# mrinmoy-iitg/SM_HPSS_MTL

Hardware: AMD Instinct MI355X
Metric: clips/sec HPSS+MTL-CNN fwd (1s@16kHz) (higher is better)
Workload: dtype f32

## Files before the change

sm_hpss_mtl_amd/csrc/smh_median.hip:

```cpp
#include <cstdlib>

#include "smh_median_kernel.h"
#include "smh_median_split.h"

namespace smh_median {

const Entry kPairs[] = {
    SMH_MEDIAN_E2(21, 11) SMH_MEDIAN_E2(17, 17)
    SMH_MEDIAN_E2(11, 11) SMH_MEDIAN_E2(11, 21) SMH_MEDIAN_E2(11, 31) SMH_MEDIAN_E2(11, 41) SMH_MEDIAN_E2(11, 51)
    SMH_MEDIAN_E2(21, 21) SMH_MEDIAN_E2(21, 31) SMH_MEDIAN_E2(21, 41) SMH_MEDIAN_E2(21, 51)
    SMH_MEDIAN_E2(31, 11) SMH_MEDIAN_E2(31, 21) SMH_MEDIAN_E2(31, 31) SMH_MEDIAN_E2(31, 41) SMH_MEDIAN_E2(31, 51)
    SMH_MEDIAN_E2(41, 11) SMH_MEDIAN_E2(41, 21) SMH_MEDIAN_E2(41, 31) SMH_MEDIAN_E2(41, 41) SMH_MEDIAN_E2(41, 51)
    SMH_MEDIAN_E2(51, 11) SMH_MEDIAN_E2(51, 21) SMH_MEDIAN_E2(51, 31) SMH_MEDIAN_E2(51, 41) SMH_MEDIAN_E2(51, 51)};

KernelFn find_pair_kernel(int lh, int lp) {
    for (const Entry &e : kPairs)
        if (e.lh == lh && e.lp == lp) return e.fn;
    return nullptr;
}

}

namespace {

// ... 105 lines not shown
    if (best < 0) return false;
    if (const char *ev = getenv("SMH_MEDIAN_SEG")) {
        int a = 0, b = 0;
        if (sscanf(ev, "%d,%d", &a, &b) == 2 && (!lh || a >= 1) && (!lp || b >= 1) &&
            waves(K, lh ? a : 0) + waves(nt, lp ? b : 0) <= maxwaves)
            bh = lh ? a : 0, bp = lp ? b : 0;
    }
    p->nsh = bh, p->nsp = bp, p->nwh = waves(K, bh), p->nwp = waves(nt, bp);
    return true;
}

int launch_small(const float *S, int B, int K, int T, int w, int along_t, float *out, hipStream_t st) {
    const size_t total = (size_t)B * K * T;
    const int bs = 256;
    hipLaunchKernelGGL(median_small_kernel, dim3((unsigned)((total + bs - 1) / bs)), dim3(bs), 0, st, S, out, K, T, w,
                       along_t, total);
    return smh::launch_status("median_small_kernel");
}

enum Family { kFamCopy = 0, kFamSmall = 1, kFamSplit = 2, kFamPersist = 3, kFamDeleteInsert = 4, kFamTwoSingles = 5 };
struct Route {
    int family, layout;
    Plan plan;
    KernelFn fn;
    const SplitEntry *se;
    const PersistEntry *pe;
    int n_cu;
};

int launch_route(int B, int K, int T, int lh, int lp, int harm_tmajor, Route *r) {
    *r = Route{};
    r->layout = harm_tmajor;
    r->fn = (lh && lp) ? find_pair_kernel(lh, lp) : find_single_kernel(lh, lp);
    if (!r->fn) return smh::set_error(SMH_E_INVALID, "no median kernel for (l_harm,l_perc)=(%d,%d)", lh, lp);
    Plan p;
    int rc = make_plan(K, T, lh, lp, &p);
    if (rc) return rc;
    static const bool no_split = getenv("SMH_MEDIAN_NOSPLIT") != nullptr;
    bool want_persist = (lh > 17 || lp > 17);
    if (const char *ev = getenv("SMH_MEDIAN_PERSIST")) want_persist = atoi(ev) != 0;
    int pthreads = 512;
    if (const char *ev = getenv("SMH_MEDIAN_PTHREADS")) pthreads = atoi(ev);
    if (const PersistEntry *pe = (no_split || !want_persist || !(lh && lp)) ? nullptr : find_persist_kernel(lh, lp, pthreads)) {
        static int n_cu = 0;
        if (n_cu == 0) {
            int dev = 0;
            SMH_CHECK_HIP(hipGetDevice(&dev));
            SMH_CHECK_HIP(hipDeviceGetAttribute(&n_cu, hipDeviceAttributeMultiprocessorCount, dev));
        }
        const int tile_bytes = persist_tile_bytes(K, T);
        const int g = T & 63;
        const bool conflict_free = (T & 1) || (g % 4 == 2);
        Plan q = p;
        if (p.ntiles == 1 && conflict_free && 2 * tile_bytes <= smh::kLdsBytesPerCU && B >= 2 * n_cu &&
            make_split_roles(K, T, lh, lp, pe->threads / 64, &q)) {
            r->family = kFamPersist, r->plan = q, r->pe = pe, r->n_cu = n_cu;
            return SMH_OK;
        }
    }
    if (const SplitEntry *se = no_split ? nullptr : find_split_kernel(lh, lp)) {
        Plan q = p;
        if (make_split_roles(K, p.TT, lh, lp, se->threads / 64, &q)) {
            r->family = kFamSplit, r->plan = q, r->se = se;
            return SMH_OK;
        }
    }
    if (harm_tmajor == 2) r->layout = 1;
    r->family = kFamDeleteInsert, r->plan = p;
    return SMH_OK;
}

int launch_routed(const Route &r, const float *S, int B, int K, int T, float *harm, float *perc, hipStream_t st) {
    if (r.family == kFamPersist) {
        const Plan &q = r.plan;
        const int lds = 2 * persist_tile_bytes(K, T);
        SMH_CHECK_HIP(hipFuncSetAttribute((const void *)r.pe->fn, hipFuncAttributeMaxDynamicSharedMemorySize, lds));
        hipLaunchKernelGGL(r.pe->fn, dim3(r.n_cu), dim3((q.nwh + q.nwp) * 64), lds, st, S, harm, perc, B, K, T, q.nsh,
                           q.nsp, q.nwh, r.layout);
        return smh::launch_status("hpss_median_persist_kernel");
    }
    if (r.family == kFamSplit) {
        const Plan &q = r.plan;
        SMH_CHECK_HIP(hipFuncSetAttribute((const void *)r.se->fn, hipFuncAttributeMaxDynamicSharedMemorySize, (int)q.lds));
        dim3 grid(q.ntiles, B), block((q.nwh + q.nwp) * 64);
        const bool probe_noload = smh::probe_env("SMH_MEDIAN_PROBE_NOLOAD") != nullptr;
        hipLaunchKernelGGL(r.se->fn, grid, block, q.lds, st, S, harm, perc, K, T, q.TT, q.stride, q.nsh, q.nsp, q.nwh,
                           r.layout, probe_noload ? 1.f : -__builtin_inff(), __builtin_inff(), nullptr, nullptr, 0);
        return smh::launch_status("hpss_median_split_kernel");
    }
    const Plan &p = r.plan;
    SMH_CHECK_HIP(hipFuncSetAttribute((const void *)r.fn, hipFuncAttributeMaxDynamicSharedMemorySize, (int)p.lds));
    dim3 grid(p.ntiles, B), block((p.nwh + p.nwp) * 64);
    hipLaunchKernelGGL(r.fn, grid, block, p.lds, st, S, harm, perc, K, T, p.TT, p.stride, p.nsh, p.nsp, p.nwh,
                       r.layout, -__builtin_inff(), __builtin_inff());
    return smh::launch_status("hpss_median_kernel");
}

int launch(const float *S, int B, int K, int T, int lh, int lp, float *harm, float *perc, hipStream_t st,
           int harm_tmajor = 0, int *written = nullptr) {
    if (written) *written = harm_tmajor;
    Route r;
    int rc = launch_route(B, K, T, lh, lp, harm_tmajor, &r);
    if (rc) return rc;
    if (written) *written = r.layout;
    return launch_routed(r, S, B, K, T, harm, perc, st);
}

int check_args(const void *S, int B, int K, int T, int w, const char *name) {
    SMH_REQUIRE(S != nullptr || B == 0, "%s: null input", name);
    SMH_REQUIRE(B >= 0 && K >= 1 && T >= 1, "%s: bad shape B=%d K=%d T=%d", name, B, K, T);
    SMH_REQUIRE(w >= 1 && w <= SMH_MAX_MEDIAN && (w & 1), "%s: window must be odd in [1,%d], got %d", name,
                SMH_MAX_MEDIAN, w);
    SMH_REQUIRE(B <= 65535, "%s: B=%d exceeds the grid limit; split the batch", name, B);
    return SMH_OK;
}

bool fast_ok(int n, int w) { return w >= 3 && w / 2 + 4 < n; }

bool pair_fused(int K, int T, int lh, int lp) { return fast_ok(T, lh) && fast_ok(K, lp) && find_pair_kernel(lh, lp); }

int hpss_route(int B, int K, int T, int lh, int lp, int want_tmajor, Route *r) {
    if (pair_fused(K, T, lh, lp)) return launch_route(B, K, T, lh, lp, want_tmajor, r);
    *r = Route{};
    r->family = kFamTwoSingles;
    return SMH_OK;
}

int time_route(int B, int K, int T, int lh, Route *r) {
    if (lh == 1 || !fast_ok(T, lh)) {
        *r = Route{};
        r->family = lh == 1 ? kFamCopy : kFamSmall;
        return SMH_OK;
    }
    return launch_route(B, K, T, lh, 0, 0, r);
}

int time_ex_route(int B, int K, int T, int lh, int harm_layout, Route *r) {
    if (lh == 1 || !fast_ok(T, lh) || harm_layout == 0) return time_route(B, K, T, lh, r);
    return launch_route(B, K, T, lh, 0, harm_layout, r);
}

}

namespace smh_median {
int rag_tile_frames(int K, int lh, int lp, int *stride) {
    static const bool no_split = getenv("SMH_MEDIAN_NOSPLIT") != nullptr;
    if (no_split || !(lh && lp) || !find_split_kernel(lh, lp)) return 0;
    const int hh = lh / 2;
    const int budget_words = (smh::kLdsBytesPerCU / 2 - 1024) / 4;
    int maxcols = budget_words / K;
    if ((maxcols & 1) == 0) maxcols -= 1;
    int TT = (maxcols - 2 * hh) & ~3;
    if (TT < 2 * hh + 8) return 0;
    if (stride) *stride = (TT + 2 * hh) | 1;
    return TT;
}

int launch_rag(const float *d_S, float *d_harm, float *d_perc, int K, int lh, int lp, const smh_rag::Clip *d_clips,
               const smh_rag::Item *d_items, int n_items, hipStream_t st) {
    if (n_items <= 0) return SMH_OK;
    int stride = 0;
    const int TT = rag_tile_frames(K, lh, lp, &stride);
    const SplitEntry *se = TT ? find_split_kernel(lh, lp) : nullptr;
    Plan q;
    if (!se || !make_split_roles(K, TT, lh, lp, se->threads / 64, &q))
        return smh::set_error(SMH_E_INVALID, "ragged medians: no block-split kernel for (l_harm,l_perc)=(%d,%d), K=%d", lh, lp, K);
    const size_t lds = (size_t)K * stride * sizeof(float);
    SMH_CHECK_HIP(hipFuncSetAttribute((const void *)se->fn, hipFuncAttributeMaxDynamicSharedMemorySize, (int)lds));
    const unsigned grid = (unsigned)(8 * (((long long)n_items + 7) / 8));
    hipLaunchKernelGGL(se->fn, dim3(grid), dim3((q.nwh + q.nwp) * 64), lds, st, d_S, d_harm, d_perc, K, 0, TT, stride, q.nsh, q.nsp,
// ... 128 lines not shown
```

sm_hpss_mtl_amd/csrc/smh_median_split.h:

```cpp
#pragma once
#include <cstdint>
#include <type_traits>
#include <utility>

#include "smh_median_kernel.h"
#include "smh_rag.h"

namespace smh_median {

template <int W>
struct SplitTraits {
    static constexpr int H = W / 2;
    static constexpr int lo(int s) { return s - H - 1 > 0 ? s - H - 1 : 0; }
    static constexpr int hi(int s) { return s - 1 < H ? s - 1 : H; }
    static constexpr int off(int s) {
        int o = 0;
        for (int r = 1; r < s; ++r) o += hi(r) - lo(r) + 1;
        return o;
    }
    static constexpr int HIST = off(W);
};

template <int B, int E, typename F>
__device__ __forceinline__ void static_for(F &&f) {
// ... 132 lines not shown
            constexpr int i = decltype(ic)::value;
            constexpr bool has_below = i - 1 >= 0;
            constexpr bool has_above = i <= s - 2;
            constexpr int po = Tr::off(s > 1 ? s - 1 : 1), pl = Tr::lo(s > 1 ? s - 1 : 1);
            const float below = has_below ? h[has_below ? po + (i - 1) - pl : 0] : 0.f;
            const float above = has_above ? h[has_above ? po + i - pl : 0] : 0.f;
            h[Tr::off(s) + i - Tr::lo(s)] = insert_slot<has_below, has_above>(below, x, above);
        });
    });
}

template <int W, int ES>
__device__ __forceinline__ void split_median_walk_blocked(const float *line, int p0, int n_out, int n_steps, int n,
                                                          char *obase, unsigned gk16, unsigned kofs) {
    using Tr = SplitTraits<W>;
    constexpr int H = W / 2, BK = W - 1;
    float e[BK];
    float h[Tr::HIST];
    float pre[H + 1];
    const int plast = p0 + n_out - 1 + H;
    auto load_block = [&](int q0) {
        const int lo = p0 - H + q0;
        const bool interior = (lo >= 0) & (lo + BK <= n) & (lo + BK - 1 <= plast);
        if (__all(interior)) {
            const float *src = line + lo * ES;
            static_for<0, BK>([&](auto uc) { e[decltype(uc)::value] = src[decltype(uc)::value * ES]; });
        } else {
            static_for<0, BK>([&](auto uc) {
                const int pos = min(lo + decltype(uc)::value, plast);
                e[decltype(uc)::value] = line[reflect_hi(reflect_lo(pos), n) * ES];
            });
        }
    };
    load_block(0);
    build_history_b<W>(e, h);
    for (int j0 = 0; j0 < n_steps; j0 += BK) {
        load_block(j0 + BK);
        float o4[4];
        static_for<0, BK>([&](auto pc) {
            constexpr int p = decltype(pc)::value;
            constexpr int b = p + 1, a = BK - p;
            static_for_down<Tr::lo(b), Tr::hi(b) + 1>([&](auto ic) {
                constexpr int i = decltype(ic)::value;
                constexpr bool has_below = i - 1 >= 0;
                constexpr bool has_above = i <= b - 2;
                const float below = has_below ? pre[has_below ? i - 1 : 0] : 0.f;
                const float above = has_above ? pre[i] : 0.f;
                pre[i] = insert_slot<has_below, has_above>(below, e[p], above);
            });
            constexpr int i_lo = (H + 1 - b) > 0 ? (H + 1 - b) : 0;
            constexpr int i_hi = a < H + 1 ? a : H + 1;
            constexpr int ao = Tr::off(a), al = Tr::lo(a);
            float r = 0.f;
            static_for<i_lo, i_hi + 1>([&](auto ic) {
                constexpr int i = decltype(ic)::value;
                float t;
                if constexpr (i == 0) t = pre[H];
                else if constexpr (H - i < 0) t = h[ao + (i - 1) - al];
                else t = fmaxf(h[ao + (i - 1) - al], pre[H - i]);
                r = (i == i_lo) ? t : fminf(r, t);
            });
            o4[p & 3] = r;
            if constexpr ((p & 3) == 3 || p == BK - 1) {
                constexpr int cnt = (p & 3) + 1, pf = p - (p & 3);
                const int j = j0 + pf, t = p0 + j;
                char *dst = obase + (unsigned)(t >> 4) * gk16 + kofs + (unsigned)(t & 15) * 4u;
                if (cnt == 4 && (t & 3) == 0 && j + 3 < n_out) {
                    float4u v = {o4[0], o4[1], o4[2], o4[3]};
                    *reinterpret_cast<float4u *>(dst) = v;
                } else {
#pragma unroll
                    for (int c = 0; c < cnt; ++c) {
                        const int tc = t + c;
                        if (j + c < n_out)
                            *reinterpret_cast<float *>(obase + (unsigned)(tc >> 4) * gk16 + kofs + (unsigned)(tc & 15) * 4u) = o4[c];
                    }
                }
            }
        });
        if (j0 + BK < n_steps) build_history_b<W>(e, h);
    }
}

template <int LH, int LP>
struct SplitCfg {
    static constexpr int kMaxW = LH > LP ? LH : LP;
    static constexpr int kThreads = kMaxW <= 17 ? 512 : 384;
    static constexpr int kWavesPerSimd = kMaxW <= 17 ? 4 : 3;
    static constexpr int kFlatBatch = kMaxW <= 17 ? 20 : 27;
};

template <int LH, int LP>
__global__ void __launch_bounds__((SplitCfg<LH, LP>::kThreads), (SplitCfg<LH, LP>::kWavesPerSimd))
hpss_median_split_kernel(const float *__restrict__ S, float *__restrict__ harm, float *__restrict__ perc, int K, int T,
                         int TT, int stride, int nsh, int nsp, int nwh, int harm_tmajor, float probe, float,
                         const smh_rag::Clip *__restrict__ rag, const smh_rag::Item *__restrict__ items, int n_items) {
    extern __shared__ __attribute__((aligned(16))) float tile[];
    constexpr int HH = LH / 2;
    int b = blockIdx.y, tile_i = blockIdx.x;
    size_t spec_off, harm_off;
    if (rag) {
        const unsigned total = (unsigned)n_items, per_xcd = (total + 7u) >> 3;
        const unsigned j = blockIdx.x >> 3, n = (blockIdx.x & 7u) * per_xcd + j;
        if (j >= per_xcd || n >= total) return;
        const smh_rag::Item item = items[n];
        b = item.clip, tile_i = item.tile;
        T = rag[b].T;
        spec_off = (size_t)rag[b].spec_off, harm_off = (size_t)rag[b].harm_off;
    } else {
        spec_off = (size_t)b * K * T;
        harm_off = harm_tmajor == 2 ? (size_t)b * ((T + 15) >> 4) * K * 16 : spec_off;
    }
    const int t0 = tile_i * TT;
    const int t1 = min(T, t0 + TT);
    const int c0 = max(0, t0 - HH), c1 = min(T, t1 + HH);
    const int ncols = c1 - c0;
    const float *Sb = S + spec_off;
    const int wave = threadIdx.x >> 6, lane = threadIdx.x & 63;
    const int nwaves = blockDim.x >> 6;

    constexpr int kFlatBatch = SplitCfg<LH, LP>::kFlatBatch;
    if (probe > 0.f) {
        for (int i = threadIdx.x; i < K * stride; i += blockDim.x) tile[i] = (float)((i * 2654435761u) >> 8) * (1.0f / 16777216.f);
    } else if (TT >= T && ((K * T) & 1) == 0 && K * T <= kFlatBatch * 2 * (int)blockDim.x) {
        const int n2 = (K * T) >> 1;
        const float2v *src = reinterpret_cast<const float2v *>(Sb);
        const unsigned magic = 0xFFFFFFFFu / (unsigned)T + 1u;
        const int extra = stride - T;
        float2v v[kFlatBatch];
#pragma unroll
        for (int r = 0; r < kFlatBatch; ++r) {
            const int idx = r * (int)blockDim.x + (int)threadIdx.x;
            v[r] = __builtin_nontemporal_load(src + min(idx, n2 - 1));
        }
#pragma unroll
        for (int r = 0; r < kFlatBatch; ++r) {
            const int idx = r * (int)blockDim.x + (int)threadIdx.x;
            if (idx < n2) {
                const unsigned g = 2u * (unsigned)idx;
                const unsigned k0 = __umulhi(g, magic), k1 = __umulhi(g + 1u, magic);
                tile[g + k0 * extra] = v[r].x;
                tile[g + 1u + k1 * extra] = v[r].y;
            }
        }
    } else if (((T | c0 | ncols) & 1) == 0 && ncols <= 128) {
        constexpr int kRowBatch = 6;
        const int n2 = ncols >> 1;
        for (int k0 = wave; k0 < K; k0 += nwaves * kRowBatch) {
            float2v v[kRowBatch];
#pragma unroll
            for (int r = 0; r < kRowBatch; ++r) {
                const int k = min(k0 + r * nwaves, K - 1);
                v[r] = __builtin_nontemporal_load(reinterpret_cast<const float2v *>(Sb + (size_t)k * T + c0) +
                                                  min(lane, n2 - 1));
            }
#pragma unroll
            for (int r = 0; r < kRowBatch; ++r) {
                const int k = k0 + r * nwaves;
                if (k < K && lane < n2) {
                    tile[k * stride + 2 * lane] = v[r].x;
                    tile[k * stride + 2 * lane + 1] = v[r].y;
                }
            }
        }
    } else {
        constexpr int kRowBatch = 6;
        for (int k0 = wave; k0 < K; k0 += nwaves * kRowBatch) {
            for (int cb = 0; cb < ncols; cb += 64) {
                float v[kRowBatch];
                const int c = cb + lane;
#pragma unroll
                for (int r = 0; r < kRowBatch; ++r) {
                    const int k = min(k0 + r * nwaves, K - 1);
                    v[r] = __builtin_nontemporal_load(Sb + (size_t)k * T + c0 + min(c, ncols - 1));
                }
#pragma unroll
                for (int r = 0; r < kRowBatch; ++r) {
                    const int k = k0 + r * nwaves;
                    if (k < K && c < ncols) tile[k * stride + c] = v[r];
                }
            }
        }
    }
    __syncthreads();

    const int nt = t1 - t0;
    if (wave < nwh) {
        if constexpr (LH > 0) {
            const int id = wave * 64 + lane;
            if (id < K * nsh) {
                const int sg = id / K, k = id - sg * K;
                const int seglen = (nt + nsh - 1) / nsh;
                const int ts = t0 + sg * seglen;
                const int te = min(t1, ts + seglen);
                if (ts < te) {
                    const float *row = tile + k * stride - c0;
                    char *ob = reinterpret_cast<char *>(harm + harm_off);
                    if (harm_tmajor == 2)
                        split_median_walk_blocked<LH, 1>(row, ts, te - ts, seglen, T, ob, (unsigned)K * 64u, (unsigned)k * 64u);
                    else if (harm_tmajor)
                        split_median_walk<LH, 1, kStridedPlain>(row, 1, ts, te - ts, seglen, T, ob,
                                                                (unsigned)(ts * K + k) * 4u, (unsigned)K * 4u);
                    else
                        split_median_walk<LH, 1, kStridedPlain>(row, 1, ts, te - ts, seglen, T, ob,
                                                                (unsigned)(k * T + ts) * 4u, 4u);
                }
            }
        }
    } else {
        if constexpr (LP > 0) {
            const int id = (wave - nwh) * 64 + lane;
            if (id < nt * nsp) {
                const int sg = id / nt, tt = id - sg * nt;
                const int seglen = (K + nsp - 1) / nsp;
                const int ks = sg * seglen;
                const int ke = min(K, ks + seglen);
                if (ks < ke) {
                    const float *col = tile + (t0 + tt - c0);
                    split_median_walk<LP, 0, kStridedStream>(col, stride, ks, ke - ks, seglen, K,
                                                             reinterpret_cast<char *>(perc + spec_off),
                                                             (unsigned)(ks * T + t0 + tt) * 4u, (unsigned)T * 4u);
                }
            }
        }
    }
}

__host__ __device__ constexpr int persist_tile_bytes(int K, int T) { return ((K * T * 4 + 16) + 1023) & ~1023; }

template <int LH, int LP, int THREADS>
__global__ void __launch_bounds__(THREADS, (THREADS / 256))
hpss_median_persist_kernel(const float *__restrict__ S, float *__restrict__ harm, float *__restrict__ perc, int B, int K,
                           int T, int nsh, int nsp, int nwh, int harm_tmajor) {
    extern __shared__ __attribute__((aligned(16))) char lds[];
    const int tile_bytes = persist_tile_bytes(K, T);
    const int wave = threadIdx.x >> 6, lane = threadIdx.x & 63;
    const int nwaves = blockDim.x >> 6;
    const size_t clip_bytes = (size_t)K * T * 4;

    auto issue_load = [&](int b, int buf) {
        const char *src = reinterpret_cast<const char *>(S) + (size_t)b * clip_bytes;
        const int mis = (int)(reinterpret_cast<uintptr_t>(src) & 15);
        src -= mis;
        const int nchunks = ((int)clip_bytes + mis + 15) >> 4;
        char *dst = lds + buf * tile_bytes;
        for (int i = wave; i * 64 < nchunks; i += nwaves) {
            const int c = i * 64 + lane;
            if (c < nchunks)
                __builtin_amdgcn_global_load_lds(
                    (const __attribute__((address_space(1))) void *)(src + (size_t)c * 16),
                    (__attribute__((address_space(3))) void *)(dst + i * 1024), 16, 0, 0);
        }
    };

    int b = blockIdx.x;
    if (b >= B) return;
    issue_load(b, 0);
    for (int it = 0; b < B; b += gridDim.x, ++it) {
        const int cur = it & 1;
        asm volatile("s_waitcnt vmcnt(0)" ::: "memory");
        __syncthreads();
        if (b + (int)gridDim.x < B) issue_load(b + gridDim.x, cur ^ 1);
        const int mis = (int)((reinterpret_cast<uintptr_t>(S) + (size_t)b * clip_bytes) & 15);
        const float *tile = reinterpret_cast<const float *>(lds + cur * tile_bytes + mis);
        if (wave < nwh) {
            const int id = wave * 64 + lane;
            if (id < K * nsh) {
                const int sg = id / K, k = id - sg * K;
                const int seglen = (T + nsh - 1) / nsh;
                const int ts = sg * seglen;
                const int te = min(T, ts + seglen);
                if (ts < te) {
                    const float *row = tile + k * T;
                    char *ob = reinterpret_cast<char *>(harm + (size_t)b * K * T);
                    if (harm_tmajor == 2)
                        split_median_walk_blocked<LH, 1>(row, ts, te - ts, seglen, T,
                                                         reinterpret_cast<char *>(harm + (size_t)b * ((T + 15) >> 4) * K * 16),
                                                         (unsigned)K * 64u, (unsigned)k * 64u);
                    else if (harm_tmajor)
                        split_median_walk<LH, 1, kStridedPlain>(row, 1, ts, te - ts, seglen, T, ob,
                                                                (unsigned)(ts * K + k) * 4u, (unsigned)K * 4u);
                    else
                        split_median_walk<LH, 1, kStridedPlain>(row, 1, ts, te - ts, seglen, T, ob,
                                                                (unsigned)(k * T + ts) * 4u, 4u);
                }
            }
        } else {
            const int id = (wave - nwh) * 64 + lane;
            if (id < T * nsp) {
                const int sg = id / T, tt = id - sg * T;
                const int seglen = (K + nsp - 1) / nsp;
                const int ks = sg * seglen;
                const int ke = min(K, ks + seglen);
                if (ks < ke)
                    split_median_walk<LP, 0, kStridedStream>(tile + tt, T, ks, ke - ks, seglen, K,
                                                             reinterpret_cast<char *>(perc + (size_t)b * K * T),
                                                             (unsigned)(ks * T + tt) * 4u, (unsigned)T * 4u);
            }
        }
    }
}

using PersistFn = void (*)(const float *, float *, float *, int, int, int, int, int, int, int);
struct PersistEntry {
    int lh, lp, threads;
    PersistFn fn;
};
const PersistEntry *find_persist_kernel(int lh, int lp, int threads);

constexpr int kSplitMaxWindow = 21;

using SplitFn = void (*)(const float *, float *, float *, int, int, int, int, int, int, int, int, float, float,
                         const smh_rag::Clip *, const smh_rag::Item *, int);
struct SplitEntry {
    int lh, lp, threads;
    SplitFn fn;
};
const SplitEntry *find_split_kernel(int lh, int lp);

}
```

sm_hpss_mtl_amd/csrc/smh_median_split.hip:

```cpp
#include "smh_median_split.h"

namespace smh_median {

#define SMH_SPLIT_E2(a, b) {a, b, SplitCfg<a, b>::kThreads, hpss_median_split_kernel<a, b>},
#define SMH_SPLIT_SINGLE(w) SMH_SPLIT_E2(w, 0) SMH_SPLIT_E2(0, w)

const SplitEntry kSplit[] = {
    SMH_SPLIT_E2(21, 11) SMH_SPLIT_E2(17, 17) SMH_SPLIT_E2(11, 11) SMH_SPLIT_E2(11, 21) SMH_SPLIT_E2(21, 21)
    SMH_SPLIT_SINGLE(3) SMH_SPLIT_SINGLE(5) SMH_SPLIT_SINGLE(7) SMH_SPLIT_SINGLE(9) SMH_SPLIT_SINGLE(11)
    SMH_SPLIT_SINGLE(13) SMH_SPLIT_SINGLE(15) SMH_SPLIT_SINGLE(17) SMH_SPLIT_SINGLE(19) SMH_SPLIT_SINGLE(21)};

const SplitEntry *find_split_kernel(int lh, int lp) {
    for (const SplitEntry &e : kSplit)
        if (e.lh == lh && e.lp == lp) return &e;
    return nullptr;
}

#define SMH_PERSIST_E3(a, b, t) {a, b, t, hpss_median_persist_kernel<a, b, t>},
#define SMH_PERSIST_E2(a, b) SMH_PERSIST_E3(a, b, 512) SMH_PERSIST_E3(a, b, 768)
const PersistEntry kPersist[] = {SMH_PERSIST_E2(21, 11) SMH_PERSIST_E2(17, 17) SMH_PERSIST_E2(11, 11)
                                 SMH_PERSIST_E2(11, 21) SMH_PERSIST_E2(21, 21) SMH_PERSIST_E3(17, 17, 1024)};

const PersistEntry *find_persist_kernel(int lh, int lp, int threads) {
    for (const PersistEntry &e : kPersist)
        if (e.lh == lh && e.lp == lp && e.threads == threads) return &e;
    return nullptr;
}

}
```

sm_hpss_mtl_amd/csrc/smh_stft.hip:

```cpp
#include <cstdint>
#include <cstdio>
#include <cstdlib>

#include "smh_common.h"
#include "smh_rag.h"

namespace {

constexpr int kThreads = 256;

struct StftArgs {
    int n_samples, n_fft, hop, M, K, T, tt;
    int n_stages;
    int radix[smh::kMaxFftStages];
    float inv_nb[smh::kMaxFftStages];
    float inv_ns[smh::kMaxFftStages];
    int tmul[smh::kMaxFftStages];
    float inv_tt;
    int B, xcd_tiles;
};

__device__ __forceinline__ float2 cmul(float2 a, float2 b) {
    return make_float2(a.x * b.x - a.y * b.y, a.x * b.y + a.y * b.x);
}
// ... 225 lines not shown

__device__ __forceinline__ void pk_dft4(v2 &a, v2 &b, v2 &c, v2 &d) {
    const v2 s0 = a + c, d0 = a - c, s1 = b + d, bd = b - d;
    a = s0 + s1;
    b = sub_i(d0, bd);
    c = s0 - s1;
    d = add_i(d0, bd);
}
__device__ __forceinline__ void pk_dft8(v2 *v) {
    v2 e0 = v[0], e1 = v[2], e2 = v[4], e3 = v[6];
    v2 o0 = v[1], o1 = v[3], o2 = v[5], o3 = v[7];
    pk_dft4(e0, e1, e2, e3);
    pk_dft4(o0, o1, o2, o3);
    const float h = 0.70710678118654752440f;
    const v2 u1 = sub_i(o1, o1);
    const v2 u3 = add_i(o3, o3);
    v[0] = e0 + o0, v[4] = e0 - o0;
    v[1] = e1 + h * u1, v[5] = e1 - h * u1;
    v[2] = sub_i(e2, o2), v[6] = add_i(e2, o2);
    v[3] = e3 - h * u3, v[7] = e3 + h * u3;
}
__device__ __forceinline__ void pk_dft5(v2 *v) {
    const float c1 = 0.30901699437494742f, c2 = -0.80901699437494742f;
    const float s1 = 0.95105651629515357f, s2 = 0.58778525229247313f;
    const v2 t1 = v[1] + v[4], t2 = v[2] + v[3], t3 = v[1] - v[4], t4 = v[2] - v[3];
    const v2 a1 = v[0] + c1 * t1 + c2 * t2, a2 = v[0] + c2 * t1 + c1 * t2;
    const v2 b1 = s1 * t3 + s2 * t4, b2 = s2 * t3 - s1 * t4;
    v[0] = v[0] + t1 + t2;
    v[1] = sub_i(a1, b1), v[4] = add_i(a1, b1);
    v[2] = sub_i(a2, b2), v[3] = add_i(a2, b2);
}
__device__ __forceinline__ void pk_dft25(v2 *x) {
    v2 t[5][5];
#pragma unroll
    for (int b = 0; b < 5; ++b) {
        v2 u[5] = {x[b], x[5 + b], x[10 + b], x[15 + b], x[20 + b]};
        pk_dft5(u);
#pragma unroll
        for (int c = 0; c < 5; ++c) {
            if (b * c == 0) {
                t[c][b] = u[c];
            } else {
                const double ang = -6.283185307179586476925 * (double)(b * c) / 25.0;
                t[c][b] = cmulp_s(u[c], v2{(float)__builtin_cos(ang), (float)__builtin_sin(ang)});
            }
        }
    }
#pragma unroll
    for (int c = 0; c < 5; ++c) {
        pk_dft5(t[c]);
#pragma unroll
        for (int d = 0; d < 5; ++d) x[c + 5 * d] = t[c][d];
    }
}

__device__ __forceinline__ void dft25(float2 *x) {
    float2 t[5][5];
#pragma unroll
    for (int b = 0; b < 5; ++b) {
        float2 u[5] = {x[b], x[5 + b], x[10 + b], x[15 + b], x[20 + b]};
        dft<5>(u);
#pragma unroll
        for (int c = 0; c < 5; ++c) {
            if (b * c == 0) {
                t[c][b] = u[c];
            } else {
                const double ang = -6.283185307179586476925 * (double)(b * c) / 25.0;
                t[c][b] = cmul(u[c], make_float2((float)__builtin_cos(ang), (float)__builtin_sin(ang)));
            }
        }
    }
#pragma unroll
    for (int c = 0; c < 5; ++c) {
        dft<5>(t[c]);
#pragma unroll
        for (int d = 0; d < 5; ++d) x[c + 5 * d] = t[c][d];
    }
}

template <int ROW>
__global__ void __launch_bounds__(512, 4)
stft400_kernel(const float *__restrict__ audio, const float *__restrict__ window, const float2 *__restrict__ twM,
               const float2 *__restrict__ tw2M, float *__restrict__ S, int n_samples, int hop, int T, int F, int probe, int B,
               int ntiles, const smh_rag::Clip *__restrict__ rag, const smh_rag::Item *__restrict__ items) {
    constexpr int M = 200, K = 201;
    extern __shared__ __attribute__((aligned(16))) float2 lds[];
    v2 *tw = reinterpret_cast<v2 *>(lds);
    v2 *tw2 = tw + 8 * ROW;
    v2 *win2 = tw2 + (M + 2);
    v2 *Z = win2 + 8 * ROW;
    auto column = [&](int it, int f, int n2) { return ROW == 25 ? n2 : n2 + 25 * (f - (it & ~15) / 25); };
    int b = blockIdx.y, tile = blockIdx.x;
    size_t clip_off, spec_off;
    if (rag) {
        const unsigned total = (unsigned)B, per_xcd = (total + 7u) >> 3;
        const unsigned j = blockIdx.x >> 3, n = (blockIdx.x & 7u) * per_xcd + j;
        if (j >= per_xcd || n >= total) return;
        const smh_rag::Item item = items[n];
        b = item.clip, tile = item.tile;
        T = rag[b].T;
        clip_off = (size_t)rag[b].audio_off, spec_off = (size_t)rag[b].spec_off;
    } else {
        if (ntiles > 0) {
            const unsigned total = (unsigned)B * (unsigned)ntiles, per_xcd = (total + 7u) >> 3;
            const unsigned j = blockIdx.x >> 3, n = (blockIdx.x & 7u) * per_xcd + j;
            if (j >= per_xcd || n >= total) return;
            b = (int)(n / (unsigned)ntiles), tile = (int)(n - (unsigned)b * (unsigned)ntiles);
        }
        clip_off = (size_t)b * n_samples, spec_off = (size_t)b * K * T;
    }
    const int t0 = tile * F, tid = threadIdx.x;
    const int nf = min(F, T - t0);
    const int nthr = blockDim.x;
    const float *clip = audio + clip_off + (size_t)t0 * hop;
    const int dq1 = nthr / 25, dr1 = nthr - dq1 * 25;
    constexpr int kRounds1 = 3;
    const bool ahead = 25 * nf <= kRounds1 * nthr;
    v2 au[kRounds1][8];
    int fr_[kRounds1], n2_[kRounds1], col_[kRounds1];
    if (ahead) {
        int f = tid / 25, n2 = tid - (tid / 25) * 25;
#pragma unroll
        for (int r = 0; r < kRounds1; ++r) {
            fr_[r] = f, n2_[r] = n2, col_[r] = column(tid + r * nthr, f, n2);
            const v2 *fr = reinterpret_cast<const v2 *>(clip + (unsigned)(min(f, nf - 1) * hop));
#pragma unroll
            for (int n1 = 0; n1 < 8; ++n1) au[r][n1] = fr[25 * n1 + n2];
            n2 += dr1;
            const int carry = n2 >= 25 ? 1 : 0;
            n2 -= 25 * carry;
            f += dq1 + carry;
        }
    }
    for (int i = tid; i < 8 * ROW; i += nthr) {
        const int k1 = i / ROW, j = i - ROW * k1, n2 = j < 25 ? j : j - 25;
        tw[i] = reinterpret_cast<const v2 *>(twM)[n2 * k1];
        win2[i] = reinterpret_cast<const v2 *>(window)[25 * k1 + n2];
    }
    for (int i = tid; i <= M; i += nthr) tw2[i] = reinterpret_cast<const v2 *>(tw2M)[i];
    __syncthreads();

    auto butterfly1 = [&](v2 (&v)[8], int f, int n2, int j) {
#pragma unroll
        for (int n1 = 0; n1 < 8; ++n1) v[n1] = v[n1] * win2[ROW * n1 + j];
        pk_dft8(v);
        v2 *zf = Z + f * kMP400 + n2;
        zf[0] = v[0];
#pragma unroll
        for (int k1 = 1; k1 < 8; ++k1) zf[k1 * 25] = cmulp(v[k1], tw[ROW * k1 + j]);
    };
    if (ahead) {
#pragma unroll
        for (int r = 0; r < kRounds1; ++r)
            if (fr_[r] < nf) butterfly1(au[r], fr_[r], n2_[r], col_[r]);
    } else {
        int it = tid;
        for (int f = tid / 25, n2 = tid - (tid / 25) * 25; f < nf; it += nthr) {
            const v2 *fr = reinterpret_cast<const v2 *>(clip + (unsigned)(f * hop));
            v2 v[8];
#pragma unroll
            for (int n1 = 0; n1 < 8; ++n1) v[n1] = fr[25 * n1 + n2];
            butterfly1(v, f, n2, column(it, f, n2));
            n2 += dr1;
            const int carry = n2 >= 25 ? 1 : 0;
            n2 -= 25 * carry;
            f += dq1 + carry;
        }
    }
    __syncthreads();
    {
        const int k1 = tid / nf, f = tid - k1 * nf;
        const bool live = k1 < 8;
        v2 x[25];
        if (live) {
            const v2 *zf = Z + f * kMP400 + k1 * 25;
#pragma unroll
            for (int n2 = 0; n2 < 25; ++n2) x[n2] = zf[n2];
        }
        __syncthreads();
        if (live) {
            pk_dft25(x);
            v2 *zo = Z + f * kMP400 + k1;
#pragma unroll
            for (int k2 = 0; k2 < 25; ++k2) zo[8 * k2] = x[k2];
        }
    }
    __syncthreads();
    float *Sb = S + spec_off + t0;
    const int dq = nthr / nf, dr = nthr - dq * nf;
    int k = tid / nf, f = tid - k * nf;
    for (; k <= M / 2; ) {
        const v2 *zf = Z + f * kMP400;
        const v2 A = zf[k], Bz = zf[k == 0 ? 0 : M - k];
        const v2 e = add_conj(A, Bz), d = sub_conj(A, Bz);
        const v2 g = cmulp(d, tw2[k]);
        {
            const v2 x = sub_i(e, g);
            const float v = 0.5f * mag(x.x, x.y);
            if (!probe || v == -1.f) Sb[(unsigned)(k * T + f)] = v;
        }
        if (k != M / 2) {
            const v2 x = add_i(e, g);
            const float v = 0.5f * mag(x.x, x.y);
            if (!probe || v == -1.f) Sb[(unsigned)((M - k) * T + f)] = v;
        }
        f += dr;
        const int carry = f >= nf ? 1 : 0;
        f -= carry * nf;
        k += dq + carry;
    }
}

}

namespace {
bool stft400_ok(const smh_ctx *ctx) {
    return ctx->cfg.n_fft == 400 && ctx->M == 200 && ctx->cfg.win_length <= 400 && (ctx->cfg.hop % 2) == 0 && !getenv("SMH_STFT_GENERIC");
}
void generic_args(const smh_ctx *ctx, StftArgs &a) {
    a.n_fft = ctx->cfg.n_fft, a.hop = ctx->cfg.hop, a.M = ctx->M, a.K = ctx->K;
    a.n_stages = ctx->n_stages;
    for (int i = 0; i < smh::kMaxFftStages; ++i) {
        a.radix[i] = i < ctx->n_stages ? ctx->radix[i] : 1;
        a.inv_nb[i] = (float)a.radix[i] / (float)a.M;
    }
    for (int i = 0, ns = 1; i < smh::kMaxFftStages; ++i) {
        a.inv_ns[i] = 1.0f / (float)ns;
        a.tmul[i] = a.M / (ns * a.radix[i]) > 0 ? a.M / (ns * a.radix[i]) : 0;
        ns *= a.radix[i];
        if (ns > a.M) ns = a.M;
    }
}
constexpr int kRagFramesGeneric = 16;
int stft_route(const smh_ctx *ctx, const float *d_audio, int B, int n_samples) {
    if (ctx->stft_f64) return 2;
    return stft400_ok(ctx) && ((n_samples % 2) == 0 || B == 1) && (reinterpret_cast<uintptr_t>(d_audio) % 8) == 0 ? 1 : 0;
}
}

extern "C" int smh_internal_stft_route(const smh_ctx *ctx, const float *d_audio, int B, int n_samples) {
    return ctx ? stft_route(ctx, d_audio, B, n_samples) : -1;
}

namespace smh_stft {
int rag_frames(const smh_ctx *ctx, bool aligned8) {
    if (ctx->stft_f64) return rag_frames_f64();
    return stft400_ok(ctx) && aligned8 ? kRagFrames : kRagFramesGeneric;
}

int launch_rag(const smh_ctx *ctx, const float *d_audio, float *d_S, const smh_rag::Clip *d_clips, const smh_rag::Item *d_items,
               int n_items, bool aligned8, hipStream_t st) {
    if (n_items <= 0) return SMH_OK;
    if (ctx->stft_f64) return launch_rag_f64(ctx, d_audio, d_S, d_clips, d_items, n_items, st);
    const unsigned grid = (unsigned)(8 * (((long long)n_items + 7) / 8));
    if (stft400_ok(ctx) && aligned8) {
        const int F = kRagFrames;
        const size_t lds = sizeof(float2) * (8 * 25 + 202 + 8 * 25 + (size_t)F * kMP400);
        SMH_CHECK_HIP(hipFuncSetAttribute((const void *)stft400_kernel<25>, hipFuncAttributeMaxDynamicSharedMemorySize, (int)lds));
        hipLaunchKernelGGL(stft400_kernel<25>, dim3(grid), dim3(256), lds, st, d_audio, ctx->d_window, ctx->d_twM, ctx->d_tw2M, d_S, 0,
                           ctx->cfg.hop, 0, F, 0, n_items, 0, d_clips, d_items);
        return smh::launch_status("stft400_kernel (ragged)");
    }
    StftArgs a;
    generic_args(ctx, a);
    a.n_samples = 0, a.T = 0, a.tt = kRagFramesGeneric, a.inv_tt = 1.0f / (float)a.tt;
    const int MP = a.M + (a.M >> 4) + 2;
    const size_t lds = sizeof(float2) * ((size_t)a.M + (a.M + 1) + 2 * (size_t)a.tt * MP);
    SMH_REQUIRE(lds <= 150 * 1024, "ragged STFT: n_fft=%d too large for the LDS FFT", a.n_fft);
    SMH_CHECK_HIP(hipFuncSetAttribute((const void *)stft_mag_kernel, hipFuncAttributeMaxDynamicSharedMemorySize, (int)lds));
    a.B = n_items, a.xcd_tiles = 0;
    hipLaunchKernelGGL(stft_mag_kernel, dim3(grid), dim3(kThreads), lds, st, a, d_audio, ctx->d_window, ctx->d_twM, ctx->d_tw2M, d_S,
                       d_clips, d_items);
    return smh::launch_status("stft_mag_kernel (ragged)");
}
}

extern "C" int smh_stft_mag_f32(const smh_ctx *ctx, const float *d_audio, int B, int n_samples, float *d_S,
                                void *stream) {
    SMH_REQUIRE(ctx && (d_audio || B == 0) && (d_S || B == 0), "smh_stft_mag_f32: null argument");
    SMH_REQUIRE(B >= 0 && B <= 65535, "smh_stft_mag_f32: B=%d out of range", B);
    const int T = smh_num_frames(n_samples, ctx->cfg.n_fft, ctx->cfg.hop);
    SMH_REQUIRE(T >= 1, "smh_stft_mag_f32: clip of %d samples is shorter than n_fft=%d", n_samples, ctx->cfg.n_fft);
    if (B == 0) return SMH_OK;
    const int route = stft_route(ctx, d_audio, B, n_samples);
    if (route == 2) return smh_stft::launch_f64(ctx, d_audio, B, n_samples, T, d_S, (hipStream_t)stream);
    if (route == 1) {
        int maxf = 20, nthreads = 256;
        if (const char *ev = getenv("SMH_STFT_FRAMES")) sscanf(ev, "%d,%d", &maxf, &nthreads);
        if (nthreads != 512) nthreads = 256;
        if (maxf < 1) maxf = 1;
        if (maxf > nthreads / 8) maxf = nthreads / 8;
        const int ntiles = (T + maxf - 1) / maxf;
        const int F = (T + ntiles - 1) / ntiles;
        int row = 25;
        if (const char *ev = smh::probe_env("SMH_STFT_ROW")) row = atoi(ev) == 40 ? 40 : 25;
        const size_t lds = sizeof(float2) * (8 * row + 202 + 8 * row + (size_t)F * kMP400);
        auto kernel = row == 40 ? stft400_kernel<40> : stft400_kernel<25>;
        SMH_CHECK_HIP(hipFuncSetAttribute((const void *)kernel, hipFuncAttributeMaxDynamicSharedMemorySize, (int)lds));
        const int nt = (T + F - 1) / F;
        bool by_xcd = true;
        if (const char *ev = getenv("SMH_STFT_XCD")) by_xcd = atoi(ev) != 0;
        if ((long long)B * nt >= (1ll << 31) - 8) by_xcd = false;
        dim3 grid(nt, B), block(nthreads);
        if (by_xcd) grid = dim3((unsigned)(8 * (((long long)B * nt + 7) / 8)), 1);
        const int probe = smh::probe_env("SMH_STFT_PROBE_NOSTORE") ? 1 : 0;
        hipLaunchKernelGGL(kernel, grid, block, lds, (hipStream_t)stream, d_audio, ctx->d_window, ctx->d_twM,
                           ctx->d_tw2M, d_S, n_samples, ctx->cfg.hop, T, F, probe, B, by_xcd ? nt : 0, nullptr, nullptr);
        return smh::launch_status("stft400_kernel");
    }
    StftArgs a;
    generic_args(ctx, a);
    a.n_samples = n_samples, a.T = T;
    const int max_tt = 16;
    const int ntiles = (T + max_tt - 1) / max_tt;
    a.tt = (T + ntiles - 1) / ntiles;
    a.inv_tt = 1.0f / (float)a.tt;
    const int MP = a.M + (a.M >> 4) + 2;
    const size_t lds = sizeof(float2) * ((size_t)a.M + (a.M + 1) + 2 * (size_t)a.tt * MP);
    SMH_REQUIRE(lds <= 150 * 1024, "smh_stft_mag_f32: n_fft=%d too large for the LDS FFT", a.n_fft);
    SMH_REQUIRE((size_t)a.tt * a.K < (1u << 20), "smh_stft_mag_f32: tile too large");
    SMH_CHECK_HIP(hipFuncSetAttribute((const void *)stft_mag_kernel, hipFuncAttributeMaxDynamicSharedMemorySize,
                                      (int)lds));
    const int ntg = (T + a.tt - 1) / a.tt;
    bool xcd_grid = (long long)B * ntg < (1ll << 31) - 8;
    if (const char *ev = getenv("SMH_STFT_XCD")) xcd_grid = xcd_grid && atoi(ev) != 0;
    a.B = B, a.xcd_tiles = xcd_grid ? ntg : 0;
    dim3 grid(ntg, B), block(kThreads);
    if (xcd_grid) grid = dim3((unsigned)(8 * (((long long)B * ntg + 7) / 8)), 1);
    hipLaunchKernelGGL(stft_mag_kernel, grid, block, lds, (hipStream_t)stream, a, d_audio, ctx->d_window, ctx->d_twM,
                       ctx->d_tw2M, d_S, nullptr, nullptr);
    return smh::launch_status("stft_mag_kernel");
}
```

Before: 2.672 million.

## Stage median clip via LDS DMA and pair STFT frames for vector stores

The split median kernel gains a variant that copies the whole clip into LDS with global_load_lds DMA when a single tile covers the clip, replacing per-thread register staging with a padded stride. The STFT400 kernel adds a paired-frame mode that packs even and odd frames so the magnitude output is written as float2 stores. It also adds a fixed-assignment path that keeps window and twiddle values in registers instead of staging them in LDS. These aim to cut load and store instruction counts and LDS setup barriers, at the cost of an unpadded LDS layout (possible bank conflicts) and more code variants.

```diff
diff --git a/sm_hpss_mtl_amd/csrc/smh_median.hip b/sm_hpss_mtl_amd/csrc/smh_median.hip
--- a/sm_hpss_mtl_amd/csrc/smh_median.hip
+++ b/sm_hpss_mtl_amd/csrc/smh_median.hip
@@ -211,10 +211,17 @@
     if (r.family == kFamSplit) {
         const Plan &q = r.plan;
         SMH_CHECK_HIP(hipFuncSetAttribute((const void *)r.se->fn, hipFuncAttributeMaxDynamicSharedMemorySize, (int)q.lds));
+        SMH_CHECK_HIP(hipFuncSetAttribute((const void *)r.se->fn_dma, hipFuncAttributeMaxDynamicSharedMemorySize, (int)q.lds));
         dim3 grid(q.ntiles, B), block((q.nwh + q.nwp) * 64);
         const bool probe_noload = smh::probe_env("SMH_MEDIAN_PROBE_NOLOAD") != nullptr;
-        hipLaunchKernelGGL(r.se->fn, grid, block, q.lds, st, S, harm, perc, K, T, q.TT, q.stride, q.nsh, q.nsp, q.nwh,
-                           r.layout, probe_noload ? 1.f : -__builtin_inff(), __builtin_inff(), nullptr, nullptr, 0);
+        const char *ev = getenv("SMH_MEDIAN_DMA_STAGE");
+        const size_t clip_bytes = (size_t)K * T * sizeof(float);
+        const uintptr_t s0 = reinterpret_cast<uintptr_t>(S);
+        const size_t align = (s0 % 16 == 0 && clip_bytes % 16 == 0) ? 16 : (s0 % 8 == 0 && clip_bytes % 8 == 0) ? 8 : 4;
+        const bool dma = !(ev && atoi(ev) == 0) && !probe_noload && q.ntiles == 1 && q.TT >= T && s0 % 4 == 0 &&
+                         ((T & 1) || ((T & 63) % 4 == 2)) && dma_stage_bytes(clip_bytes, align) <= q.lds;
+        hipLaunchKernelGGL(dma ? r.se->fn_dma : r.se->fn, grid, block, q.lds, st, S, harm, perc, K, T, q.TT, dma ? T : q.stride, q.nsh,
+                           q.nsp, q.nwh, r.layout, probe_noload ? 1.f : -__builtin_inff(), __builtin_inff(), nullptr, nullptr, 0);
         return smh::launch_status("hpss_median_split_kernel");
     }
     const Plan &p = r.plan;
diff --git a/sm_hpss_mtl_amd/csrc/smh_median_split.h b/sm_hpss_mtl_amd/csrc/smh_median_split.h
--- a/sm_hpss_mtl_amd/csrc/smh_median_split.h
+++ b/sm_hpss_mtl_amd/csrc/smh_median_split.h
@@ -238,6 +238,21 @@
     }
 }
 
+__device__ __forceinline__ int stage_clip_dma(const char *src, int bytes, char *dst, int wave, int nwaves, int lane) {
+    const int mis = (int)(reinterpret_cast<uintptr_t>(src) & 15);
+    src -= mis;
+    const int nchunks = (bytes + mis + 15) >> 4;
+    for (int i = wave; i * 64 < nchunks; i += nwaves) {
+        const int c = i * 64 + lane;
+        if (c < nchunks)
+            __builtin_amdgcn_global_load_lds(
+                (const __attribute__((address_space(1))) void *)(src + (size_t)c * 16),
+                (__attribute__((address_space(3))) void *)(dst + i * 1024), 16, 0, 0);
+    }
+    return mis;
+}
+__host__ __device__ constexpr size_t dma_stage_bytes(size_t bytes, size_t align) { return (bytes + (16 - align) + 15) & ~(size_t)15; }
+
 template <int LH, int LP>
 struct SplitCfg {
     static constexpr int kMaxW = LH > LP ? LH : LP;
@@ -246,12 +261,13 @@
     static constexpr int kFlatBatch = kMaxW <= 17 ? 20 : 27;
 };
 
-template <int LH, int LP>
+template <int LH, int LP, bool DMA = false>
 __global__ void __launch_bounds__((SplitCfg<LH, LP>::kThreads), (SplitCfg<LH, LP>::kWavesPerSimd))
 hpss_median_split_kernel(const float *__restrict__ S, float *__restrict__ harm, float *__restrict__ perc, int K, int T,
                          int TT, int stride, int nsh, int nsp, int nwh, int harm_tmajor, float probe, float,
                          const smh_rag::Clip *__restrict__ rag, const smh_rag::Item *__restrict__ items, int n_items) {
-    extern __shared__ __attribute__((aligned(16))) float tile[];
+    extern __shared__ __attribute__((aligned(16))) float tile_lds[];
+    const float *tile = tile_lds;
     constexpr int HH = LH / 2;
     int b = blockIdx.y, tile_i = blockIdx.x;
     size_t spec_off, harm_off;
@@ -276,8 +292,12 @@
     const int nwaves = blockDim.x >> 6;
 
     constexpr int kFlatBatch = SplitCfg<LH, LP>::kFlatBatch;
-    if (probe > 0.f) {
-        for (int i = threadIdx.x; i < K * stride; i += blockDim.x) tile[i] = (float)((i * 2654435761u) >> 8) * (1.0f / 16777216.f);
+    if constexpr (DMA) {
+        const int mis = stage_clip_dma(reinterpret_cast<const char *>(Sb), K * T * 4, reinterpret_cast<char *>(tile_lds), wave, nwaves, lane);
+        tile = reinterpret_cast<const float *>(reinterpret_cast<const char *>(tile_lds) + mis);
+        asm volatile("s_waitcnt vmcnt(0)" ::: "memory");
+    } else if (probe > 0.f) {
+        for (int i = threadIdx.x; i < K * stride; i += blockDim.x) tile_lds[i] = (float)((i * 2654435761u) >> 8) * (1.0f / 16777216.f);
     } else if (TT >= T && ((K * T) & 1) == 0 && K * T <= kFlatBatch * 2 * (int)blockDim.x) {
         const int n2 = (K * T) >> 1;
         const float2v *src = reinterpret_cast<const float2v *>(Sb);
@@ -295,8 +315,8 @@
             if (idx < n2) {
                 const unsigned g = 2u * (unsigned)idx;
                 const unsigned k0 = __umulhi(g, magic), k1 = __umulhi(g + 1u, magic);
-                tile[g + k0 * extra] = v[r].x;
-                tile[g + 1u + k1 * extra] = v[r].y;
+                tile_lds[g + k0 * extra] = v[r].x;
+                tile_lds[g + 1u + k1 * extra] = v[r].y;
             }
         }
     } else if (((T | c0 | ncols) & 1) == 0 && ncols <= 128) {
@@ -314,8 +334,8 @@
             for (int r = 0; r < kRowBatch; ++r) {
                 const int k = k0 + r * nwaves;
                 if (k < K && lane < n2) {
-                    tile[k * stride + 2 * lane] = v[r].x;
-                    tile[k * stride + 2 * lane + 1] = v[r].y;
+                    tile_lds[k * stride + 2 * lane] = v[r].x;
+                    tile_lds[k * stride + 2 * lane + 1] = v[r].y;
                 }
             }
         }
@@ -333,7 +353,7 @@
 #pragma unroll
                 for (int r = 0; r < kRowBatch; ++r) {
                     const int k = k0 + r * nwaves;
-                    if (k < K && c < ncols) tile[k * stride + c] = v[r];
+                    if (k < K && c < ncols) tile_lds[k * stride + c] = v[r];
                 }
             }
         }
@@ -395,18 +415,7 @@
     const size_t clip_bytes = (size_t)K * T * 4;
 
     auto issue_load = [&](int b, int buf) {
-        const char *src = reinterpret_cast<const char *>(S) + (size_t)b * clip_bytes;
-        const int mis = (int)(reinterpret_cast<uintptr_t>(src) & 15);
-        src -= mis;
-        const int nchunks = ((int)clip_bytes + mis + 15) >> 4;
-        char *dst = lds + buf * tile_bytes;
-        for (int i = wave; i * 64 < nchunks; i += nwaves) {
-            const int c = i * 64 + lane;
-            if (c < nchunks)
-                __builtin_amdgcn_global_load_lds(
-                    (const __attribute__((address_space(1))) void *)(src + (size_t)c * 16),
-                    (__attribute__((address_space(3))) void *)(dst + i * 1024), 16, 0, 0);
-        }
+        stage_clip_dma(reinterpret_cast<const char *>(S) + (size_t)b * clip_bytes, (int)clip_bytes, lds + buf * tile_bytes, wave, nwaves, lane);
     };
 
     int b = blockIdx.x;
@@ -470,7 +479,7 @@
                          const smh_rag::Clip *, const smh_rag::Item *, int);
 struct SplitEntry {
     int lh, lp, threads;
-    SplitFn fn;
+    SplitFn fn, fn_dma;
 };
 const SplitEntry *find_split_kernel(int lh, int lp);
 
diff --git a/sm_hpss_mtl_amd/csrc/smh_median_split.hip b/sm_hpss_mtl_amd/csrc/smh_median_split.hip
--- a/sm_hpss_mtl_amd/csrc/smh_median_split.hip
+++ b/sm_hpss_mtl_amd/csrc/smh_median_split.hip
@@ -2,7 +2,7 @@
 
 namespace smh_median {
 
-#define SMH_SPLIT_E2(a, b) {a, b, SplitCfg<a, b>::kThreads, hpss_median_split_kernel<a, b>},
+#define SMH_SPLIT_E2(a, b) {a, b, SplitCfg<a, b>::kThreads, hpss_median_split_kernel<a, b>, hpss_median_split_kernel<a, b, true>},
 #define SMH_SPLIT_SINGLE(w) SMH_SPLIT_E2(w, 0) SMH_SPLIT_E2(0, w)
 
 const SplitEntry kSplit[] = {
diff --git a/sm_hpss_mtl_amd/csrc/smh_stft.hip b/sm_hpss_mtl_amd/csrc/smh_stft.hip
--- a/sm_hpss_mtl_amd/csrc/smh_stft.hip
+++ b/sm_hpss_mtl_amd/csrc/smh_stft.hip
@@ -331,7 +331,7 @@
 __global__ void __launch_bounds__(512, 4)
 stft400_kernel(const float *__restrict__ audio, const float *__restrict__ window, const float2 *__restrict__ twM,
                const float2 *__restrict__ tw2M, float *__restrict__ S, int n_samples, int hop, int T, int F, int probe, int B,
-               int ntiles, const smh_rag::Clip *__restrict__ rag, const smh_rag::Item *__restrict__ items) {
+               int ntiles, int pairs, const smh_rag::Clip *__restrict__ rag, const smh_rag::Item *__restrict__ items) {
     constexpr int M = 200, K = 201;
     extern __shared__ __attribute__((aligned(16))) float2 lds[];
     v2 *tw = reinterpret_cast<v2 *>(lds);
@@ -362,12 +362,32 @@
     const int nf = min(F, T - t0);
     const int nthr = blockDim.x;
     const float *clip = audio + clip_off + (size_t)t0 * hop;
+    float *Sb = S + spec_off + t0;
     const int dq1 = nthr / 25, dr1 = nthr - dq1 * 25;
+    const int nh = nf >> 1;
+    const bool pair3 = pairs && ((nf | t0 | T) & 1) == 0 && (reinterpret_cast<uintptr_t>(Sb) & 7) == 0;
+    auto slot_frame = [&](int s) { return pair3 ? (s < nh ? 2 * s : 2 * (s - nh) + 1) : s; };
+    auto frame_slot = [&](int f) { return pair3 ? (f >> 1) + (f & 1) * nh : f; };
     constexpr int kRounds1 = 3;
-    const bool ahead = 25 * nf <= kRounds1 * nthr;
+    const bool fixed = pairs && nf <= kRounds1 * dq1;
+    const bool ahead = !fixed && 25 * nf <= kRounds1 * nthr;
     v2 au[kRounds1][8];
     int fr_[kRounds1], n2_[kRounds1], col_[kRounds1];
-    if (ahead) {
+    v2 wr[8], tr[8];
+    if (fixed) {
+        const int fg = tid / 25, n2 = tid - fg * 25;
+#pragma unroll
+        for (int r = 0; r < kRounds1; ++r) {
+            const int f = slot_frame(min(fg + r * dq1, nf - 1));
+            const v2 *fr = reinterpret_cast<const v2 *>(clip + (unsigned)(f * hop));
+#pragma unroll
+            for (int n1 = 0; n1 < 8; ++n1) au[r][n1] = fr[25 * n1 + n2];
+        }
+#pragma unroll
+        for (int n1 = 0; n1 < 8; ++n1) wr[n1] = reinterpret_cast<const v2 *>(window)[25 * n1 + n2];
+#pragma unroll
+        for (int k1 = 1; k1 < 8; ++k1) tr[k1] = reinterpret_cast<const v2 *>(twM)[n2 * k1];
+    } else if (ahead) {
         int f = tid / 25, n2 = tid - (tid / 25) * 25;
 #pragma unroll
         for (int r = 0; r < kRounds1; ++r) {
@@ -381,41 +401,57 @@
             f += dq1 + carry;
         }
     }
-    for (int i = tid; i < 8 * ROW; i += nthr) {
-        const int k1 = i / ROW, j = i - ROW * k1, n2 = j < 25 ? j : j - 25;
-        tw[i] = reinterpret_cast<const v2 *>(twM)[n2 * k1];
-        win2[i] = reinterpret_cast<const v2 *>(window)[25 * k1 + n2];
-    }
-    for (int i = tid; i <= M; i += nthr) tw2[i] = reinterpret_cast<const v2 *>(tw2M)[i];
-    __syncthreads();
-
-    auto butterfly1 = [&](v2 (&v)[8], int f, int n2, int j) {
-#pragma unroll
-        for (int n1 = 0; n1 < 8; ++n1) v[n1] = v[n1] * win2[ROW * n1 + j];
-        pk_dft8(v);
-        v2 *zf = Z + f * kMP400 + n2;
-        zf[0] = v[0];
-#pragma unroll
-        for (int k1 = 1; k1 < 8; ++k1) zf[k1 * 25] = cmulp(v[k1], tw[ROW * k1 + j]);
-    };
-    if (ahead) {
-#pragma unroll
-        for (int r = 0; r < kRounds1; ++r)
-            if (fr_[r] < nf) butterfly1(au[r], fr_[r], n2_[r], col_[r]);
+    const v2 t2 = reinterpret_cast<const v2 *>(tw2M)[min(tid, M)];
+    if (fixed) {
+#pragma unroll
+        for (int r = 0; r < kRounds1; ++r) {
+            const int fg = tid / 25, s = fg + r * dq1;
+            if (fg < dq1 && s < nf) {
+#pragma unroll
+                for (int n1 = 0; n1 < 8; ++n1) au[r][n1] = au[r][n1] * wr[n1];
+                pk_dft8(au[r]);
+                v2 *zf = Z + s * kMP400 + (tid - fg * 25);
+                zf[0] = au[r][0];
+#pragma unroll
+                for (int k1 = 1; k1 < 8; ++k1) zf[k1 * 25] = cmulp(au[r][k1], tr[k1]);
+            }
+        }
     } else {
-        int it = tid;
-        for (int f = tid / 25, n2 = tid - (tid / 25) * 25; f < nf; it += nthr) {
-            const v2 *fr = reinterpret_cast<const v2 *>(clip + (unsigned)(f * hop));
-            v2 v[8];
-#pragma unroll
-            for (int n1 = 0; n1 < 8; ++n1) v[n1] = fr[25 * n1 + n2];
-            butterfly1(v, f, n2, column(it, f, n2));
-            n2 += dr1;
-            const int carry = n2 >= 25 ? 1 : 0;
-            n2 -= 25 * carry;
-            f += dq1 + carry;
-        }
-    }
+        for (int i = tid; i < 8 * ROW; i += nthr) {
+            const int k1 = i / ROW, j = i - ROW * k1, n2 = j < 25 ? j : j - 25;
+            tw[i] = reinterpret_cast<const v2 *>(twM)[n2 * k1];
+            win2[i] = reinterpret_cast<const v2 *>(window)[25 * k1 + n2];
+        }
+        __syncthreads();
+        auto butterfly1 = [&](v2 (&v)[8], int f, int n2, int j) {
+#pragma unroll
+            for (int n1 = 0; n1 < 8; ++n1) v[n1] = v[n1] * win2[ROW * n1 + j];
+            pk_dft8(v);
+            v2 *zf = Z + frame_slot(f) * kMP400 + n2;
+            zf[0] = v[0];
+#pragma unroll
+            for (int k1 = 1; k1 < 8; ++k1) zf[k1 * 25] = cmulp(v[k1], tw[ROW * k1 + j]);
+        };
+        if (ahead) {
+#pragma unroll
+            for (int r = 0; r < kRounds1; ++r)
+                if (fr_[r] < nf) butterfly1(au[r], fr_[r], n2_[r], col_[r]);
+        } else {
+            int it = tid;
+            for (int f = tid / 25, n2 = tid - (tid / 25) * 25; f < nf; it += nthr) {
+                const v2 *fr = reinterpret_cast<const v2 *>(clip + (unsigned)(f * hop));
+                v2 v[8];
+#pragma unroll
+                for (int n1 = 0; n1 < 8; ++n1) v[n1] = fr[25 * n1 + n2];
+                butterfly1(v, f, n2, column(it, f, n2));
+                n2 += dr1;
+                const int carry = n2 >= 25 ? 1 : 0;
+                n2 -= 25 * carry;
+                f += dq1 + carry;
+            }
+        }
+    }
+    if (tid <= M) tw2[tid] = t2;
     __syncthreads();
     {
         const int k1 = tid / nf, f = tid - k1 * nf;
@@ -435,24 +471,41 @@
         }
     }
     __syncthreads();
-    float *Sb = S + spec_off + t0;
+    auto untangle = [](v2 A, v2 Bz, v2 w, float &lo, float &hi) {
+        const v2 e = add_conj(A, Bz), d = sub_conj(A, Bz);
+        const v2 g = cmulp(d, w);
+        const v2 x = sub_i(e, g);
+        lo = 0.5f * mag(x.x, x.y);
+        const v2 y = add_i(e, g);
+        hi = 0.5f * mag(y.x, y.y);
+    };
+    if (pair3) {
+        const int dq = nthr / nh, dr = nthr - dq * nh;
+        int k = tid / nh, fp = tid - k * nh;
+        for (; k <= M / 2;) {
+            const v2 *z0 = Z + fp * kMP400, *z1 = z0 + nh * kMP400;
+            const int kb = k == 0 ? 0 : M - k;
+            const v2 w = tw2[k];
+            float2 lo, hi;
+            untangle(z0[k], z0[kb], w, lo.x, hi.x);
+            untangle(z1[k], z1[kb], w, lo.y, hi.y);
+            if (!probe || lo.x == -1.f) *reinterpret_cast<float2 *>(Sb + (unsigned)(k * T + 2 * fp)) = lo;
+            if (k != M / 2 && (!probe || hi.x == -1.f)) *reinterpret_cast<float2 *>(Sb + (unsigned)((M - k) * T + 2 * fp)) = hi;
+            fp += dr;
+            const int carry = fp >= nh ? 1 : 0;
+            fp -= carry * nh;
+            k += dq + carry;
+        }
+        return;
+    }
     const int dq = nthr / nf, dr = nthr - dq * nf;
     int k = tid / nf, f = tid - k * nf;
     for (; k <= M / 2; ) {
         const v2 *zf = Z + f * kMP400;
-        const v2 A = zf[k], Bz = zf[k == 0 ? 0 : M - k];
-        const v2 e = add_conj(A, Bz), d = sub_conj(A, Bz);
-        const v2 g = cmulp(d, tw2[k]);
-        {
-            const v2 x = sub_i(e, g);
-            const float v = 0.5f * mag(x.x, x.y);
-            if (!probe || v == -1.f) Sb[(unsigned)(k * T + f)] = v;
-        }
-        if (k != M / 2) {
-            const v2 x = add_i(e, g);
-            const float v = 0.5f * mag(x.x, x.y);
-            if (!probe || v == -1.f) Sb[(unsigned)((M - k) * T + f)] = v;
-        }
+        float lo, hi;
+        untangle(zf[k], zf[k == 0 ? 0 : M - k], tw2[k], lo, hi);
+        if (!probe || lo == -1.f) Sb[(unsigned)(k * T + f)] = lo;
+        if (k != M / 2 && (!probe || hi == -1.f)) Sb[(unsigned)((M - k) * T + f)] = hi;
         f += dr;
         const int carry = f >= nf ? 1 : 0;
         f -= carry * nf;
@@ -465,6 +518,10 @@
 namespace {
 bool stft400_ok(const smh_ctx *ctx) {
     return ctx->cfg.n_fft == 400 && ctx->M == 200 && ctx->cfg.win_length <= 400 && (ctx->cfg.hop % 2) == 0 && !getenv("SMH_STFT_GENERIC");
+}
+int stft400_pairs() {
+    const char *ev = getenv("SMH_STFT_PAIRS");
+    return ev && atoi(ev) == 0 ? 0 : 1;
 }
 void generic_args(const smh_ctx *ctx, StftArgs &a) {
     a.n_fft = ctx->cfg.n_fft, a.hop = ctx->cfg.hop, a.M = ctx->M, a.K = ctx->K;
@@ -507,7 +564,7 @@
         const size_t lds = sizeof(float2) * (8 * 25 + 202 + 8 * 25 + (size_t)F * kMP400);
         SMH_CHECK_HIP(hipFuncSetAttribute((const void *)stft400_kernel<25>, hipFuncAttributeMaxDynamicSharedMemorySize, (int)lds));
         hipLaunchKernelGGL(stft400_kernel<25>, dim3(grid), dim3(256), lds, st, d_audio, ctx->d_window, ctx->d_twM, ctx->d_tw2M, d_S, 0,
-                           ctx->cfg.hop, 0, F, 0, n_items, 0, d_clips, d_items);
+                           ctx->cfg.hop, 0, F, 0, n_items, 0, stft400_pairs(), d_clips, d_items);
         return smh::launch_status("stft400_kernel (ragged)");
     }
     StftArgs a;
@@ -540,7 +597,9 @@
         if (maxf < 1) maxf = 1;
         if (maxf > nthreads / 8) maxf = nthreads / 8;
         const int ntiles = (T + maxf - 1) / maxf;
-        const int F = (T + ntiles - 1) / ntiles;
+        int F = (T + ntiles - 1) / ntiles;
+        const int pairs = stft400_pairs();
+        if (pairs && T % 2 == 0 && F % 2 != 0 && F < maxf) ++F;
         int row = 25;
         if (const char *ev = smh::probe_env("SMH_STFT_ROW")) row = atoi(ev) == 40 ? 40 : 25;
         const size_t lds = sizeof(float2) * (8 * row + 202 + 8 * row + (size_t)F * kMP400);
@@ -554,7 +613,7 @@
         if (by_xcd) grid = dim3((unsigned)(8 * (((long long)B * nt + 7) / 8)), 1);
         const int probe = smh::probe_env("SMH_STFT_PROBE_NOSTORE") ? 1 : 0;
         hipLaunchKernelGGL(kernel, grid, block, lds, (hipStream_t)stream, d_audio, ctx->d_window, ctx->d_twM,
-                           ctx->d_tw2M, d_S, n_samples, ctx->cfg.hop, T, F, probe, B, by_xcd ? nt : 0, nullptr, nullptr);
+                           ctx->d_tw2M, d_S, n_samples, ctx->cfg.hop, T, F, probe, B, by_xcd ? nt : 0, pairs, nullptr, nullptr);
         return smh::launch_status("stft400_kernel");
     }
     StftArgs a;
```

Measured after the change: 2.743 million, median of 6. +2.7%, better.
